# rockstaedt/DecentralOPF.jl

Hardware: AMD Instinct MI355X
Metric: agent_subproblem_updates_per_sec (higher is better)
Workload: dtype f64

## Files before the change

decentralopf.jl_amd/csrc/sto_lean.h:

```cpp
#pragma once
#include <type_traits>

namespace dopf {

template <class Tp>
__device__ __forceinline__ Tp *lz_at(Tp *base, unsigned byte_off)
{
    return reinterpret_cast<Tp *>(reinterpret_cast<char *>(const_cast<typename std::remove_const<Tp>::type *>(base)) + byte_off);
}

template <int CTRL>
__device__ __forceinline__ double lz_dpp(double x)
{
    const int lo = __builtin_amdgcn_update_dpp(0, __double2loint(x), CTRL, 0xF, 0xF, true);
    const int hi = __builtin_amdgcn_update_dpp(0, __double2hiint(x), CTRL, 0xF, 0xF, true);
    return __hiloint2double(hi, lo);
}
template <int CTRL>
__device__ __forceinline__ int lz_dppi(int x)
{
    return __builtin_amdgcn_update_dpp(0, x, CTRL, 0xF, 0xF, true);
}
template <int CTRL, bool ZERO_OK>
__device__ __forceinline__ double lz_dpp_id(double x, double idv)
{
    if (ZERO_OK) return lz_dpp<CTRL>(x);
    const int lo = __builtin_amdgcn_update_dpp(__double2loint(idv), __double2loint(x), CTRL, 0xF, 0xF, false);
    const int hi = __builtin_amdgcn_update_dpp(__double2hiint(idv), __double2hiint(x), CTRL, 0xF, 0xF, false);
    return __hiloint2double(hi, lo);
}

template <int CTRL, int RM>
__device__ __forceinline__ double lz_dpp_rm(double x, double idv)
{
    const int lo = __builtin_amdgcn_update_dpp(__double2loint(idv), __double2loint(x), CTRL, RM, 0xF, false);
    const int hi = __builtin_amdgcn_update_dpp(__double2hiint(idv), __double2hiint(x), CTRL, RM, 0xF, false);
    return __hiloint2double(hi, lo);
}

template <int LPS>
__device__ __forceinline__ double lz_prev(double x)
{
    if (LPS <= 16) return lz_dpp<0x111>(x);
    return lz_dpp<0x138>(x);
}
template <int LPS>
__device__ __forceinline__ double lz_next(double x)
{
    if (LPS <= 16) return lz_dpp<0x101>(x);
    return lz_dpp<0x130>(x);
}
template <int LPS>
__device__ __forceinline__ int lz_previ(int x)
{
    if (LPS <= 16) return lz_dppi<0x111>(x);
    return lz_dppi<0x138>(x);
}

template <int LPS>
__device__ __forceinline__ void lz_seg_sum2(double k, double &a, double &b)
{
#define DOPF_LZ_STEP(CTRL)                                                           \
    {                                                                                \
        const double pa = lz_dpp<CTRL>(a), pb = lz_dpp<CTRL>(b), pk = lz_dpp_id<CTRL, (LPS <= 16)>(k, 1.0); \
        a = fma(pa, k, a); b = fma(pb, k, b); k *= pk;                                \
    }
    DOPF_LZ_STEP(0x111)
    if (LPS >= 4) DOPF_LZ_STEP(0x112)
    if (LPS >= 8) DOPF_LZ_STEP(0x114)
    if (LPS >= 16) DOPF_LZ_STEP(0x118)
    if (LPS == 32) DOPF_LZ_STEP(0x142)
#undef DOPF_LZ_STEP
    if (LPS >= 64) {
#define DOPF_LZ_STEP64(CTRL, RM)                                                     \
        {                                                                            \
            const double pa = lz_dpp_rm<CTRL, RM>(a, 0.0), pb = lz_dpp_rm<CTRL, RM>(b, 0.0), pk = lz_dpp_rm<CTRL, RM>(k, 1.0); \
            a = fma(pa, k, a); b = fma(pb, k, b); k *= pk;                            \
        }
        DOPF_LZ_STEP64(0x142, 0xA)
        DOPF_LZ_STEP64(0x143, 0xC)
#undef DOPF_LZ_STEP64
    }
}

template <int LPS, bool LOWER>
__device__ __forceinline__ void lz_chain_scan(double &M, double &G, int lane)
{
#define DOPF_LZ_STEP(CTRL)                                                           \
    {                                                                                \
        const double pM = lz_dpp_id<CTRL, (LPS <= 16)>(M, LOWER ? -INFINITY : INFINITY);   \
        const double pG = lz_dpp_id<CTRL, (LPS <= 16)>(G, LOWER ? INFINITY : -INFINITY);   \
        if (LOWER) { M = lz_max(M, lz_min(G, pM)); G = lz_min(G, pG); }               \
        else { M = lz_min(M, lz_max(G, pM)); G = lz_max(G, pG); }                     \
    }
    DOPF_LZ_STEP(0x101)
    if (LPS >= 4) DOPF_LZ_STEP(0x102)
    if (LPS >= 8) DOPF_LZ_STEP(0x104)
    if (LPS >= 16) DOPF_LZ_STEP(0x108)
#undef DOPF_LZ_STEP
    if (LPS >= 32) {
        const double pM = __shfl(M, (lane | 15) + 1), pG = __shfl(G, (lane | 15) + 1);
        if ((lane & 16) == 0) {
            if (LOWER) { M = lz_max(M, lz_min(G, pM)); G = lz_min(G, pG); }
            else { M = lz_min(M, lz_max(G, pM)); G = lz_max(G, pG); }
        }
    }
    if (LPS >= 64) {
        const double pM = __shfl(M, 32), pG = __shfl(G, 32);
        if ((lane & 32) == 0) {
            if (LOWER) { M = lz_max(M, lz_min(G, pM)); G = lz_min(G, pG); }
            else { M = lz_min(M, lz_max(G, pM)); G = lz_max(G, pG); }
        }
    }
}

template <int LPS>
__device__ __forceinline__ void lz_seg_maxmin(double K, double &a, double &b)
{
#define DOPF_LZ_STEP(CTRL)                                                           \
    {                                                                                \
        const double pa = lz_dpp_id<CTRL, (LPS <= 16)>(a, -INFINITY), pb = lz_dpp_id<CTRL, (LPS <= 16)>(b, INFINITY); \
        const double pK = lz_dpp_id<CTRL, (LPS <= 16)>(K, INFINITY);                   \
        a = lz_max(a, lz_min(K, pa)); b = lz_min(b, lz_max(-K, pb)); K = lz_min(K, pK); \
    }
    DOPF_LZ_STEP(0x111)
    if (LPS >= 4) DOPF_LZ_STEP(0x112)
    if (LPS >= 8) DOPF_LZ_STEP(0x114)
    if (LPS >= 16) DOPF_LZ_STEP(0x118)
    if (LPS == 32) DOPF_LZ_STEP(0x142)
#undef DOPF_LZ_STEP
    if (LPS >= 64) {
#define DOPF_LZ_STEP64(CTRL, RM)                                                     \
        {                                                                            \
            const double pa = lz_dpp_rm<CTRL, RM>(a, -INFINITY), pb = lz_dpp_rm<CTRL, RM>(b, INFINITY), pK = lz_dpp_rm<CTRL, RM>(K, INFINITY); \
            a = lz_max(a, lz_min(K, pa)); b = lz_min(b, lz_max(-K, pb)); K = lz_min(K, pK); \
        }
        DOPF_LZ_STEP64(0x142, 0xA)
        DOPF_LZ_STEP64(0x143, 0xC)
#undef DOPF_LZ_STEP64
    }
}

template <int LPS, int NCH>
__device__ __attribute__((noinline)) int sto_warm_lines_call(const DevView *self, const int blk, const int halt)
{
    return sto_warm_body<LPS, NCH, true>(*self, blk, halt);
}

template <int LPS, int NCH, bool TAIL, bool LINES = false, bool FULLT = true>
__device__ __forceinline__ int sto_lean_body(const DevView &v, const int blk, const int halt)
{
    static_assert(LPS <= 64 && NCH <= 8, "4 pattern bits per step");
    static_assert(!(TAIL && LINES), "the tail in the launch: copper plates");
    constexpr int NG = 256 / LPS, TP = LPS * NCH;
    const int T = FULLT ? TP : v.T;
    constexpr int MAXR = 16;
    constexpr int MAXN = 40;
    constexpr int BIG = 0x3fffffff;
    __shared__ double red[NG * TP];
    __shared__ double fdL[NG * TP];
    const int tid = threadIdx.x, lane = tid & 63, li = tid & (LPS - 1), grp = tid / LPS;
    const int gbase = lane & ~(LPS - 1);
    Item it;
    if (v.stoChunk > 0) { it.a0 = blk * v.stoChunk; it.a1 = min(v.S, it.a0 + v.stoChunk); it.node = 0; }
    else it = v.sto_items[blk];
    const int N = v.N;
    const double w = v.w_prox, gam = v.gamma;
    const double a0 = w + gam, ia0 = v.cp_ia, idet0 = v.cp_idet, s20 = v.cp_s2;
    const int tbase = li * NCH;
    double *nuL = red + grp * TP, *fd_ = fdL + grp * TP;
    const bool first = li == 0, last = li == LPS - 1;
#define LZ_IN(c) (FULLT || tbase + (c) < T)
#define LZ_TLAST(c) (FULLT ? (last && (c) == NCH - 1) : (tbase + (c) == T - 1))
    double lp0[NCH], kapL[NCH], iaL[NCH], idetL[NCH], s2L[NCH];
#define LZ_KAP(c) (LINES ? kapL[c] : gam)
#define LZ_AA(c) (LINES ? w + kapL[c] : a0)
#define LZ_IA(c) (LINES ? iaL[c] : ia0)
#define LZ_IDET(c) (LINES ? idetL[c] : idet0)
#define LZ_S2(c) (LINES ? s2L[c] : s20)
    if (LINES) {
        int nonlin = 0;
#pragma unroll
        for (int c = 0; c < NCH; ++c) {
            lp0[c] = 0.0; kapL[c] = gam; iaL[c] = ia0; idetL[c] = idet0; s2L[c] = s20;
            if (LZ_IN(c)) {
                const size_t at = (size_t)it.node + (size_t)N * (tbase + c);
                const int m_ = v.tb_m[at];
                const double p0_ = v.tb_psi0[at], k_ = v.tb_slope[at * (v.M2 + 1)];
                nonlin |= m_ != 0;
                lp0[c] = p0_; kapL[c] = k_;
                lin_coef(w, 1.0 / w, k_, iaL[c], idetL[c], s2L[c]);
            }
        }
        if (__syncthreads_or(nonlin)) return sto_warm_lines_call<LPS, NCH>(v.self, blk, halt);
    }

    double accQ[NCH];
    double accCost = 0.0;
    int anyFail = 0;
#pragma unroll
    for (int c = 0; c < NCH; ++c) accQ[c] = 0.0;
    __shared__ double th0L[TP];
    if (!LINES) {
        if (tid < LPS) {
#pragma unroll
            for (int c = 0; c < NCH; ++c) th0L[tbase + c] = LZ_IN(c) ? v.price[it.node + N * (tbase + c)] + gam * v.s[tbase + c] : 0.0;
        }
        __syncthreads();
    }
#ifdef DOPF_STATS
    unsigned long long st_rounds = 0, st_newton = 0, st_short = 0;
#endif
    const int nRep = (it.a1 - it.a0 + NG - 1) / NG;
    for (int rep = 0; rep < nRep; ++rep) {
        const int s = it.a0 + rep * NG + grp;
        const bool live = s < it.a1;
        const unsigned sl = live ? (unsigned)s : (unsigned)it.a0;
        const double mc = v.sto_mc[sl], pm = v.sto_pmax[sl], em = v.sto_emax[sl];
        const bool havenu = live && v.nu_valid[sl] != 0;
        double A0[NCH], B0[NCH], nuv[NCH], dq[NCH];
        double run = 0.0;
        double d0r[NCH], c0r[NCH], nur[NCH];
#pragma unroll
        for (int c = 0; c < NCH; ++c) {
            const int t = tbase + c;
            const unsigned eb = (sl * (unsigned)T + (unsigned)(LZ_IN(c) ? t : 0)) * 8u;
            d0r[c] = *lz_at(v.D, eb); c0r[c] = *lz_at(v.C, eb);
            nur[c] = *lz_at(v.nu_prev, eb);
            if (!LZ_IN(c)) { d0r[c] = 0.0; c0r[c] = 0.0; nur[c] = 0.0; }
        }
#pragma unroll
        for (int c = 0; c < NCH; ++c) {
            const int t = tbase + c;
            const double d0 = d0r[c], c0 = c0r[c], nu_st = nur[c];
            const double theta = LINES ? lp0[c] - kapL[c] * (d0 - c0) : th0L[t] - gam * (d0 - c0);
            dq[c] = c0 - d0;
            run += c0 - d0;
            A0[c] = w * d0 - mc - theta; B0[c] = w * c0 - mc + theta;
            nuv[c] = havenu ? (LINES ? nu_st : nu_st - theta) : 0.0;
            if (!LZ_IN(c)) { A0[c] = -1e300; B0[c] = -1e300; nuv[c] = 0.0; }
        }
        if (rep == 0 && halt) return -1;

        const double tolc = 1e-9 * (1.0 + em), tolE = 1e-11 * (1.0 + em), tolr = 1e-12 * (1.0 + em);
        int kind[NCH];
        {
            double inclE = run, zero_ = 0.0;
            lz_seg_sum2<LPS>(first ? 0.0 : 1.0, inclE, zero_);
            const double prevE = lz_prev<LPS>(inclE);
            double eo = first ? 0.0 : prevE;
#pragma unroll
            for (int c = 0; c < NCH; ++c) {
                eo += dq[c];
                kind[c] = !LZ_IN(c) ? 0 : (eo <= tolc ? 1 : (eo >= em - tolc ? 2 : 0));
            }
        }

        bool gdone = !live, good = false;
        double Dv[NCH], Cv[NCH], nuc[NCH];
        for (int round = 0; round < MAXR; ++round) {
#ifdef DOPF_STATS
            if (first && !gdone) ++st_rounds;
#endif
            bool en[NCH];
            double keep[NCH], pk[NCH], sb[NCH];
#define LZ_TGT(c) (kind[c] == 2 ? em : 0.0)
            int send[NCH];
            bool st0;
            {
#pragma unroll
                for (int c = 0; c < NCH; ++c) {
                    en[c] = kind[c] != 0 || LZ_TLAST(c);
                }
                const int pkd = lz_previ<LPS>(FULLT ? kind[NCH - 1] : (en[NCH - 1] ? (kind[NCH - 1] == 2 ? 2 : 1) : 0));
                st0 = first || pkd != 0;
                double run_k = 1.0;
#pragma unroll
                for (int c = 0; c < NCH; ++c) {
                    const bool stc = c == 0 ? st0 : en[c > 0 ? c - 1 : 0];
                    keep[c] = stc ? 0.0 : 1.0;
                    run_k *= keep[c];
                    pk[c] = run_k;
                    sb[c] = !stc ? 0.0 : (c == 0 ? ((!first && pkd == 2) ? em : 0.0) : LZ_TGT(c > 0 ? c - 1 : 0));
                }
                int mfirst = BIG;
#pragma unroll
                for (int c = NCH - 1; c >= 0; --c)
                    if (en[c]) mfirst = tbase + c;
                const int incl = scan_min_rev_i<LPS>(mfirst, lane);
                const int nxt = next_lane_i<LPS>(incl);
                int carry = last ? BIG : nxt;
#pragma unroll
                for (int c = NCH - 1; c >= 0; --c) {
                    if (en[c]) carry = tbase + c;
                    send[c] = carry < TP ? carry : TP - 1;
                }
#pragma unroll
                for (int c = 0; c < NCH; ++c)
                    if (en[c]) nuL[tbase + c] = kind[c] != 0 ? nuv[c] : 0.0;
                __builtin_amdgcn_wave_barrier();
#pragma unroll
                for (int c = 0; c < NCH; ++c) nuv[c] = LZ_IN(c) ? nuL[send[c]] : 0.0;
                __builtin_amdgcn_wave_barrier();
            }

            double px[NCH], ps[NCH];
            double blo[NCH], bhi[NCH];
#pragma unroll
            for (int c = 0; c < NCH; ++c) { blo[c] = -INFINITY; bhi[c] = INFINITY; }
            bool nconv = false, nfail = false;
            unsigned pat = 0u;
            bool stepped = false;
            for (int itn = 0; itn < MAXN; ++itn) {
#ifdef DOPF_STATS
                if (first && !gdone) ++st_newton;
#endif
                unsigned npat = 0u;
                double sl[NCH];
#pragma unroll
                for (int c = 0; c < NCH; ++c) {
                    double dd, cc, s1;
                    box2(LZ_AA(c), LZ_KAP(c), LZ_IA(c), LZ_IDET(c), LZ_S2(c), A0[c] - nuv[c], B0[c] + nuv[c], pm, dd, cc, s1);
                    Dv[c] = dd; Cv[c] = cc; sl[c] = s1;
                    const unsigned cD = dd <= 0.0 ? 0u : (dd >= pm ? 2u : 1u), cC = cc <= 0.0 ? 0u : (cc >= pm ? 2u : 1u);
                    npat |= (cD | (cC << 2)) << (4 * c);
                }
                const bool same = stepped && __all(npat == pat || gdone);
                pat = npat;
                if (same) {
                    bool q = false;
#pragma unroll
                    for (int c = 0; c < NCH; ++c) q = q || (en[c] && kind[c] != 0 && fabs(px[c] - LZ_TGT(c)) > tolr);
                    if (!__any(q && !gdone)) {
#ifdef DOPF_STATS
                        if (first && !gdone) ++st_short;
#endif
                        nconv = !nfail;
                        break;
                    }
                }
                {
                    double rx = 0.0, rs = 0.0;
#pragma unroll
                    for (int c = 0; c < NCH; ++c) {
                        rx = fma(rx, keep[c], (Cv[c] - Dv[c]) + sb[c]);
                        rs = fma(rs, keep[c], sl[c]);
                        px[c] = rx; ps[c] = rs;
                    }
                    double ax = rx, as = rs;
                    lz_seg_sum2<LPS>(pk[NCH - 1], ax, as);
                    const double cx = lz_prev<LPS>(ax), cs = lz_prev<LPS>(as);
#pragma unroll
                    for (int c = 0; c < NCH; ++c) { px[c] = fma(cx, pk[c], px[c]); ps[c] = fma(cs, pk[c], ps[c]); }
                }
                double res[NCH];
                bool need[NCH], flatNeed = false;
#pragma unroll
                for (int c = 0; c < NCH; ++c) {
                    res[c] = px[c] - LZ_TGT(c);
                    need[c] = en[c] && kind[c] != 0 && fabs(res[c]) > tolr;
                    flatNeed = flatNeed || (need[c] && !(ps[c] > 0.0));
                }
                if (__any(flatNeed && !gdone)) {
                    double ru = -INFINITY, rd = INFINITY;
                    double fu[NCH], fn[NCH];
#pragma unroll
                    for (int c = 0; c < NCH; ++c) {
                        double du = INFINITY, dn = INFINITY;
                        const double sh = LZ_KAP(c) * (Dv[c] - Cv[c]);
                        const double bD = A0[c] - sh, bC = -B0[c] - sh, wp = w * pm;
                        const double cand[4] = {bD, bD - wp, bC, bC + wp};
#pragma unroll
                        for (int q = 0; q < 4; ++q) {
                            const double d = cand[q] - nuv[c];
                            if (d > 0.0) du = lz_min(du, d);
                            if (d < 0.0) dn = lz_min(dn, -d);
                        }
                        if (keep[c] == 0.0) { ru = -INFINITY; rd = INFINITY; }
                        ru = lz_max(ru, -du); rd = lz_min(rd, dn);
                        fu[c] = ru; fn[c] = rd;
                    }
                    double au = ru, ad = rd;
                    lz_seg_maxmin<LPS>(pk[NCH - 1] != 0.0 ? INFINITY : -INFINITY, au, ad);
                    const double cu = lz_prev<LPS>(au), cd = lz_prev<LPS>(ad);
#pragma unroll
                    for (int c = 0; c < NCH; ++c) {
                        if (pk[c] != 0.0) { fu[c] = lz_max(fu[c], cu); fn[c] = lz_min(fn[c], cd); }
                        if (en[c] && kind[c] != 0) fd_[tbase + c] = res[c] < 0.0 ? -fu[c] : -fn[c];
                    }
                }
                bool plain = true;
#pragma unroll
                for (int c = 0; c < NCH; ++c) {
                    if (need[c]) {
                        const int t = tbase + c;
                        const double r = res[c], nu = nuv[c];
                        if (r < 0.0) blo[c] = nu; else bhi[c] = nu;
                        const bool both = blo[c] > -INFINITY && bhi[c] < INFINITY;
                        double trial;
                        bool isPlain = true;
                        if (ps[c] > 0.0) {
                            trial = nu - r * rcp64(ps[c]);
                        } else {
                            const double sd = fd_[t];
                            trial = nu + sd + copysign(1e-9 * (1.0 + fabs(nu) + fabs(sd)), sd);
                            isPlain = false;
                        }
                        if (!(trial > blo[c] && trial < bhi[c]) || (both && itn >= 8 && (itn & 1))) {
                            if (both) { trial = 0.5 * (blo[c] + bhi[c]); isPlain = false; }
                        }
                        if (trial > blo[c] && trial < bhi[c]) { nuL[t] = trial; plain = plain && isPlain; }
                        else if (both) need[c] = false;
                        else nfail = true;
                    }
                }
                bool bad = false;
#pragma unroll
                for (int c = 0; c < NCH; ++c) bad = bad || need[c];
                nfail = group_bits<LPS>(nfail, gbase) != 0ull;
                nconv = group_bits<LPS>(bad, gbase) == 0ull && !nfail;
                if (__all(gdone || nconv || nfail)) break;
                stepped = __all(plain || gdone || nconv || nfail) != 0;
                __builtin_amdgcn_wave_barrier();
#pragma unroll
                for (int c = 0; c < NCH; ++c) {
                    const double nn = LZ_IN(c) ? nuL[send[c]] : 0.0;
                    px[c] = fma(ps[c], nn - nuv[c], px[c]);
                    nuv[c] = nn;
                }
                __builtin_amdgcn_wave_barrier();
            }

            bool okk = true;
            int nkind[NCH];
            double mlo[NCH], mhi[NCH];
            {
                double rl = -INFINITY, rh = INFINITY;
                double slo[NCH], shi[NCH];
#pragma unroll
                for (int c = 0; c < NCH; ++c) {
                    const double dd = Dv[c], cc = Cv[c];
                    const double lD = fma(LZ_KAP(c), cc, A0[c]), hC = -fma(LZ_KAP(c), dd, B0[c]), apm = LZ_AA(c) * pm;
                    double lo = dd <= 0.0 ? lD : -INFINITY;
                    double hi = (dd > 0.0 && dd >= pm) ? lD - apm : INFINITY;
                    hi = lz_min(hi, cc <= 0.0 ? hC : INFINITY);
                    lo = lz_max(lo, (cc > 0.0 && cc >= pm) ? hC + apm : -INFINITY);
                    const double K = keep[c] != 0.0 ? INFINITY : -INFINITY;
                    rl = lz_max(lo, lz_min(K, rl)); rh = lz_min(hi, lz_max(-K, rh));
                    slo[c] = rl; shi[c] = rh;
                }
                double al = rl, ah = rh;
                lz_seg_maxmin<LPS>(pk[NCH - 1] != 0.0 ? INFINITY : -INFINITY, al, ah);
                const double cl = lz_prev<LPS>(al), ch = lz_prev<LPS>(ah);
#pragma unroll
                for (int c = 0; c < NCH; ++c) {
                    nkind[c] = kind[c];
                    const bool contact = en[c] && kind[c] != 0;
                    if (!contact) {
                        if (px[c] < -tolE) { okk = false; nkind[c] = 1; }
                        else if (px[c] > em + tolE) { okk = false; nkind[c] = 2; }
                    }
                    const double Kp = pk[c] != 0.0 ? INFINITY : -INFINITY;
                    const double sl_ = lz_max(slo[c], lz_min(Kp, cl)), sh_ = lz_min(shi[c], lz_max(-Kp, ch));
                    const double pt = kind[c] != 0 ? nuv[c] : 0.0;
                    const bool flat = contact && ps[c] == 0.0 && sl_ <= sh_ && nuv[c] >= sl_ - 1e-9 && nuv[c] <= sh_ + 1e-9;
                    mlo[c] = flat ? sl_ : pt; mhi[c] = flat ? sh_ : pt;
                }
            }
            {
                double Ml = -INFINITY, Gl = INFINITY, Mh = INFINITY, Gh = -INFINITY;
                if (last) { Ml = 0.0; Gl = -INFINITY; Mh = 0.0; Gh = INFINITY; }
#define LZ_EL(c) (en[c] ? mlo[c] : -INFINITY)
#define LZ_GL(c) ((!en[c] || kind[c] == 1) ? INFINITY : -INFINITY)
#define LZ_EH(c) (en[c] ? mhi[c] : INFINITY)
#define LZ_GH(c) ((!en[c] || kind[c] == 2) ? -INFINITY : INFINITY)
#pragma unroll
                for (int c = NCH - 1; c >= 0; --c) {
                    Ml = lz_max(LZ_EL(c), lz_min(LZ_GL(c), Ml)); Gl = lz_min(LZ_GL(c), Gl);
                    Mh = lz_min(LZ_EH(c), lz_max(LZ_GH(c), Mh)); Gh = lz_max(LZ_GH(c), Gh);
                }
                lz_chain_scan<LPS, true>(Ml, Gl, lane);
                lz_chain_scan<LPS, false>(Mh, Gh, lane);
                const double nextMl = lz_next<LPS>(Ml), nextMh = lz_next<LPS>(Mh);
                double flo = last ? 0.0 : nextMl, fhi = last ? 0.0 : nextMh;
#pragma unroll
                for (int c = NCH - 1; c >= 0; --c) {
                    flo = lz_max(LZ_EL(c), lz_min(LZ_GL(c), flo));
                    fhi = lz_min(LZ_EH(c), lz_max(LZ_GH(c), fhi));
                    nuc[c] = nuv[c];
                    if (en[c] && kind[c] != 0) {
                        const double tn = 1e-10 * (1.0 + lz_minabs(flo, fhi));
                        if (flo > fhi + tn) { okk = false; nkind[c] = 0; }
                        nuc[c] = lz_min(lz_max(nuv[c], flo), lz_max(flo, fhi));
                    }
                }
#undef LZ_EL
#undef LZ_GL
#undef LZ_EH
#undef LZ_GH
            }
            {
                int nrel = 0;
#pragma unroll
                for (int c = 0; c < NCH; ++c) nrel += __popcll(group_bits<LPS>(nkind[c] == 0 && kind[c] != 0, gbase));
                const bool fwd = nrel >= 1 && nrel <= 4 && !gdone;
                if (__any(fwd)) {
                    double Llo = -INFINITY, Lhi = INFINITY, Ulo = -INFINITY, Uhi = INFINITY;
#pragma unroll
                    for (int c = 0; c < NCH; ++c) {
                        if (en[c]) {
                            const double l_lo = kind[c] == 2 ? mlo[c] : -INFINITY, l_hi = kind[c] == 2 ? INFINITY : -INFINITY;
                            const double u_lo = kind[c] == 1 ? -INFINITY : INFINITY, u_hi = kind[c] == 1 ? mhi[c] : INFINITY;
                            const double a1 = clampd(Llo, l_lo, l_hi), a2 = clampd(Lhi, l_lo, l_hi);
                            const double b1 = clampd(Ulo, u_lo, u_hi), b2 = clampd(Uhi, u_lo, u_hi);
                            Llo = a1; Lhi = a2; Ulo = b1; Uhi = b2;
                        }
                    }
                    scan_clamps_fwd<LPS>(Llo, Lhi, lane);
                    scan_clamps_fwd<LPS>(Ulo, Uhi, lane);
                    const double leftL = prev_lane<LPS>(Llo), leftU = prev_lane<LPS>(Uhi);
                    double pin = first ? -INFINITY : leftL, phin = first ? INFINITY : leftU;
#pragma unroll
                    for (int c = 0; c < NCH; ++c) {
                        if (en[c]) {
                            const double glo = fmax(mlo[c], pin), ghi = fmin(mhi[c], phin);
                            const double tn = 1e-10 * (1.0 + fmin(fabs(glo), fabs(ghi)));
                            fd_[tbase + c] = glo > ghi + tn ? 1.0 : 0.0;
                            pin = kind[c] == 2 ? glo : -INFINITY;
                            phin = kind[c] == 1 ? ghi : INFINITY;
                        }
                    }
                    __builtin_amdgcn_wave_barrier();
                    const int sendNext = next_lane_i<LPS>(send[0]);
#pragma unroll
                    for (int c = 0; c < NCH; ++c) {
                        if (!LZ_TLAST(c) && en[c] && kind[c] != 0) {
                            const int sn = c + 1 < NCH ? send[c + 1 < NCH ? c + 1 : c] : sendNext;
                            if (fwd && fd_[sn] != 0.0) { okk = false; nkind[c] = 0; }
                        }
                    }
                    __builtin_amdgcn_wave_barrier();
                }
            }
            const bool cert = nconv && group_bits<LPS>(!okk, gbase) == 0ull && !(v.debugLeave && s % 3 == 0);
            bool chg = false;
#pragma unroll
            for (int c = 0; c < NCH; ++c) chg = chg || nkind[c] != kind[c];
            const bool changed = group_bits<LPS>(chg, gbase) != 0ull;

            if (!gdone && cert) {
                int s_ = s;
                asm volatile("" : "+v"(s_));
#pragma unroll
                for (int c = 0; c < NCH; ++c) {
                    if (!LZ_IN(c)) continue;
                    const unsigned eb = ((unsigned)s_ * (unsigned)T + (unsigned)(tbase + c)) * 8u;
                    *lz_at(v.D, eb) = Dv[c];
                    *lz_at(v.C, eb) = Cv[c];
                    *lz_at(v.nu_prev, eb) = LINES ? nuc[c] : nuc[c] + 0.5 * (B0[c] - A0[c] - w * dq[c]);
                    if (LINES && (v.keepDeltas || v.walk_any[tbase + c])) *lz_at(v.dltS, eb) = (Dv[c] - Cv[c]) + dq[c];
                    accQ[c] += Dv[c] - Cv[c];
                    accCost += mc * (Dv[c] + Cv[c]);
                }
                good = true;
                gdone = true;
            }
            if (!gdone && (!nconv || !changed)) gdone = true;
            if (__all(gdone)) break;
            if (!gdone) {
#pragma unroll
                for (int c = 0; c < NCH; ++c) kind[c] = nkind[c];
            }
            __builtin_amdgcn_wave_barrier();
#undef LZ_TGT
        }

        if (live && first) { v.sto_fail[s] = good ? 0 : 1; if (good) v.nu_valid[s] = 1; }
        if (live && !good && first) anyFail += 1;
        __builtin_amdgcn_wave_barrier();
    }
#ifdef DOPF_STATS
    if (st_rounds) atomicAdd(&v.st->dbg_reason[0], st_rounds);
    if (st_newton) atomicAdd(&v.st->dbg_reason[1], st_newton);
    if (st_short) atomicAdd(&v.st->dbg_events, st_short);
    if (st_rounds) atomicMax(&v.st->dbg_reason[2], st_rounds);
    if (st_newton) atomicMax(&v.st->dbg_reason[3], st_newton);
#endif

#pragma unroll
    for (int c = 0; c < NCH; ++c) {
        double x = accQ[c];
        if (LPS <= 8) x += lz_dpp<0x128>(x);
        if (LPS <= 16) x += __shfl_xor(x, 16);
        if (LPS <= 32) x += __shfl_xor(x, 32);
        accQ[c] = x;
    }
    __shared__ double wsumS[4][TP];
    __shared__ double wcostS[4];
    __shared__ int wfailS[4];
    {
        double cw = accCost;
        int fw = anyFail;
        for (int d = 32; d > 0; d >>= 1) { cw += __shfl_xor(cw, d); fw += __shfl_xor(fw, d); }
        if (lane == 0) { wcostS[tid >> 6] = cw; wfailS[tid >> 6] = fw; }
        if (lane < LPS) {
#pragma unroll
            for (int c = 0; c < NCH; ++c) wsumS[tid >> 6][tbase + c] = accQ[c];
        }
    }
    const DevView *pf = v.self;
    asm volatile("" : "+s"(pf));
    TailView tv{};
    int tpar = 0;
    if (TAIL) { tv = *pf->tailDev; tpar = pf->st->tail_par; }
    asm volatile("s_waitcnt lgkmcnt(0)\n\ts_barrier" ::: "memory");
    const int blockFail = wfailS[0] + wfailS[1] + wfailS[2] + wfailS[3];
    if (tid < LPS) {
#pragma unroll
        for (int c = 0; c < NCH; ++c) {
            const int t = tbase + c;
            if (!LZ_IN(c)) continue;
            const double sum = ((wsumS[0][t] + wsumS[1][t]) + wsumS[2][t]) + wsumS[3][t];
            if (TAIL && blockFail == 0) acc_add(tv, tpar, t, sum, tv.scaleInj);
            else if (LINES) pf->part_T[(size_t)t * pf->rowsT + it.row + 1] = sum;
            else pf->part_sinj_w[(size_t)blk * T + t] = sum;
        }
    }
    if (tid == 0) {
        const double cw = ((wcostS[0] + wcostS[1]) + wcostS[2]) + wcostS[3];
        if (TAIL && blockFail == 0) acc_add(tv, tpar, T, cw, tv.scaleCost);
        else pf->part_scost_w[blk] = cw;
        pf->item_fail[blk] = blockFail;
    }
    if (blockFail != 0) __syncthreads();
    return blockFail;
#undef LZ_IN
#undef LZ_TLAST
#undef LZ_KAP
#undef LZ_AA
#undef LZ_IA
#undef LZ_IDET
#undef LZ_S2
}

}
```

Before: 2.148 billion.

## Prefetch first storage rows and tail pointers before block barrier in lean body

The first repetition's storage rows (mc, pmax, emax, D, C, nu_prev) are loaded before the initial barrier, so their latency overlaps the price/imbalance loads and the synchronisation. Tail-view and output pointers are read early by one thread and parked in shared memory, which removes the dependent global pointer-chasing loads from the epilogue. Optional timeline stamps are added behind a compile flag. In exchange the kernel holds more live registers across the barrier, and the register-clobber trick used to reset the row registers after each iteration is fragile.

```diff
diff --git a/decentralopf.jl_amd/csrc/sto_lean.h b/decentralopf.jl_amd/csrc/sto_lean.h
--- a/decentralopf.jl_amd/csrc/sto_lean.h
+++ b/decentralopf.jl_amd/csrc/sto_lean.h
@@ -146,6 +146,20 @@
 {
     return sto_warm_body<LPS, NCH, true>(*self, blk, halt);
 }
+
+struct LzPark {
+    long long *acc;
+    double scaleInj, scaleCost;
+    double *part_sinj_w, *part_scost_w;
+    int *item_fail;
+    int accStride, tail_par;
+};
+
+#ifdef DOPF_BLOCK_STAMPS
+#define DOPF_LZ_STAMP(i) { if (threadIdx.x == 0 && blk < 4096) g_timeline[98304 + 8 * blk + (i)] = wall_clock64(); }
+#else
+#define DOPF_LZ_STAMP(i)
+#endif
 
 template <int LPS, int NCH, bool TAIL, bool LINES = false, bool FULLT = true>
 __device__ __forceinline__ int sto_lean_body(const DevView &v, const int blk, const int halt)
@@ -201,12 +215,54 @@
 #pragma unroll
     for (int c = 0; c < NCH; ++c) accQ[c] = 0.0;
     __shared__ double th0L[TP];
+    __shared__ LzPark parkL;
+    double mc, pm, em;
+    bool havenu;
+    double d0r[NCH], c0r[NCH], nur[NCH];
+#define LZ_LOAD_ROWS(sl_, live_)                                                          \
+    {                                                                                \
+        mc = v.sto_mc[sl_]; pm = v.sto_pmax[sl_]; em = v.sto_emax[sl_];              \
+        havenu = (live_) && v.nu_valid[sl_] != 0;                                    \
+        _Pragma("unroll")                                                            \
+        for (int c = 0; c < NCH; ++c) {                                              \
+            const unsigned eb = ((sl_) * (unsigned)T + (unsigned)(LZ_IN(c) ? tbase + c : 0)) * 8u; \
+            d0r[c] = *lz_at(v.D, eb); c0r[c] = *lz_at(v.C, eb);                      \
+            nur[c] = *lz_at(v.nu_prev, eb);                                          \
+            if (!LZ_IN(c)) { d0r[c] = 0.0; c0r[c] = 0.0; nur[c] = 0.0; }             \
+        }                                                                            \
+    }
     if (!LINES) {
+        double prc[NCH], imb[NCH];
+        LzPark pw{};
         if (tid < LPS) {
 #pragma unroll
-            for (int c = 0; c < NCH; ++c) th0L[tbase + c] = LZ_IN(c) ? v.price[it.node + N * (tbase + c)] + gam * v.s[tbase + c] : 0.0;
-        }
-        __syncthreads();
+            for (int c = 0; c < NCH; ++c) {
+                const int t = LZ_IN(c) ? tbase + c : 0;
+                prc[c] = v.price[it.node + N * t]; imb[c] = v.s[t];
+            }
+        }
+        if (tid == 64) {
+            if (TAIL) {
+                const TailView *tp = v.tail;
+                pw.acc = tp->acc; pw.accStride = tp->accStride; pw.scaleInj = tp->scaleInj; pw.scaleCost = tp->scaleCost;
+                pw.tail_par = v.st->tail_par;
+            }
+            pw.part_sinj_w = v.part_sinj_w; pw.part_scost_w = v.part_scost_w; pw.item_fail = v.item_fail;
+        }
+        asm volatile("" ::: "memory");
+        {
+            const int s0 = it.a0 + grp;
+            const unsigned sl0 = s0 < it.a1 ? (unsigned)s0 : (unsigned)it.a0;
+            LZ_LOAD_ROWS(sl0, s0 < it.a1)
+        }
+        asm volatile("" ::: "memory");
+        if (tid < LPS) {
+#pragma unroll
+            for (int c = 0; c < NCH; ++c) th0L[tbase + c] = LZ_IN(c) ? prc[c] + gam * imb[c] : 0.0;
+        }
+        if (tid == 64) parkL = pw;
+        DOPF_LZ_STAMP(0)
+        asm volatile("s_waitcnt lgkmcnt(0)\n\ts_barrier" ::: "memory");
     }
 #ifdef DOPF_STATS
     unsigned long long st_rounds = 0, st_newton = 0, st_short = 0;
@@ -216,19 +272,12 @@
         const int s = it.a0 + rep * NG + grp;
         const bool live = s < it.a1;
         const unsigned sl = live ? (unsigned)s : (unsigned)it.a0;
-        const double mc = v.sto_mc[sl], pm = v.sto_pmax[sl], em = v.sto_emax[sl];
-        const bool havenu = live && v.nu_valid[sl] != 0;
+        if (LINES || rep > 0) LZ_LOAD_ROWS(sl, live)
+#ifdef DOPF_BLOCK_STAMPS
+        if (rep == 0) { asm volatile("s_waitcnt vmcnt(0)" ::: "memory"); DOPF_LZ_STAMP(1) }
+#endif
         double A0[NCH], B0[NCH], nuv[NCH], dq[NCH];
         double run = 0.0;
-        double d0r[NCH], c0r[NCH], nur[NCH];
-#pragma unroll
-        for (int c = 0; c < NCH; ++c) {
-            const int t = tbase + c;
-            const unsigned eb = (sl * (unsigned)T + (unsigned)(LZ_IN(c) ? t : 0)) * 8u;
-            d0r[c] = *lz_at(v.D, eb); c0r[c] = *lz_at(v.C, eb);
-            nur[c] = *lz_at(v.nu_prev, eb);
-            if (!LZ_IN(c)) { d0r[c] = 0.0; c0r[c] = 0.0; nur[c] = 0.0; }
-        }
 #pragma unroll
         for (int c = 0; c < NCH; ++c) {
             const int t = tbase + c;
@@ -578,7 +627,13 @@
         if (live && first) { v.sto_fail[s] = good ? 0 : 1; if (good) v.nu_valid[s] = 1; }
         if (live && !good && first) anyFail += 1;
         __builtin_amdgcn_wave_barrier();
-    }
+        if (!LINES) {
+            havenu = false;
+#pragma unroll
+            for (int c = 0; c < NCH; ++c) asm volatile("" : "=v"(d0r[c]), "=v"(c0r[c]), "=v"(nur[c]));
+        }
+    }
+    DOPF_LZ_STAMP(2)
 #ifdef DOPF_STATS
     if (st_rounds) atomicAdd(&v.st->dbg_reason[0], st_rounds);
     if (st_newton) atomicAdd(&v.st->dbg_reason[1], st_newton);
@@ -609,11 +664,17 @@
         }
     }
     const DevView *pf = v.self;
-    asm volatile("" : "+s"(pf));
+    if (LINES) asm volatile("" : "+s"(pf));
+    asm volatile("s_waitcnt lgkmcnt(0)\n\ts_barrier" ::: "memory");
+    DOPF_LZ_STAMP(3)
     TailView tv{};
     int tpar = 0;
-    if (TAIL) { tv = *pf->tailDev; tpar = pf->st->tail_par; }
-    asm volatile("s_waitcnt lgkmcnt(0)\n\ts_barrier" ::: "memory");
+    double *psinj = nullptr, *pscost = nullptr;
+    int *pfail = nullptr;
+    if (!LINES && tid < LPS) {
+        if (TAIL) { tv.acc = parkL.acc; tv.accStride = parkL.accStride; tv.scaleInj = parkL.scaleInj; tv.scaleCost = parkL.scaleCost; tpar = parkL.tail_par; }
+        psinj = parkL.part_sinj_w; pscost = parkL.part_scost_w; pfail = parkL.item_fail;
+    }
     const int blockFail = wfailS[0] + wfailS[1] + wfailS[2] + wfailS[3];
     if (tid < LPS) {
 #pragma unroll
@@ -623,17 +684,21 @@
             const double sum = ((wsumS[0][t] + wsumS[1][t]) + wsumS[2][t]) + wsumS[3][t];
             if (TAIL && blockFail == 0) acc_add(tv, tpar, t, sum, tv.scaleInj);
             else if (LINES) pf->part_T[(size_t)t * pf->rowsT + it.row + 1] = sum;
-            else pf->part_sinj_w[(size_t)blk * T + t] = sum;
+            else psinj[(size_t)blk * T + t] = sum;
         }
     }
     if (tid == 0) {
         const double cw = ((wcostS[0] + wcostS[1]) + wcostS[2]) + wcostS[3];
         if (TAIL && blockFail == 0) acc_add(tv, tpar, T, cw, tv.scaleCost);
-        else pf->part_scost_w[blk] = cw;
-        pf->item_fail[blk] = blockFail;
-    }
+        else if (LINES) pf->part_scost_w[blk] = cw;
+        else pscost[blk] = cw;
+        if (LINES) pf->item_fail[blk] = blockFail;
+        else pfail[blk] = blockFail;
+    }
+    DOPF_LZ_STAMP(4)
     if (blockFail != 0) __syncthreads();
     return blockFail;
+#undef LZ_LOAD_ROWS
 #undef LZ_IN
 #undef LZ_TLAST
 #undef LZ_KAP
```

After: 2.125 billion. 0.989x the previous value.
